# qhy991/llama.cpp-quant-gemm

Measured on AMD Instinct MI355X. Metric: effective TFLOPS + GB/s, Q4_0×Q8_1 GEMV M=1 N=K=4096; NMSE vs FP32, higher is better.
Workload: dtype int8; 1 GPU; q4_0_q8_1_gemv; M=1, N=4096, K=4096, rows_per_gpu=4096, weight_copies=64, parallelism=row-shard x1, launch=hipGraph, kernel_algo=1

## Files before the change

### include/qg/qg.h

```cpp
#ifndef QG_QG_H
#define QG_QG_H

#include <stddef.h>
#include <stdint.h>

#ifdef __cplusplus
extern "C" {
#endif

typedef struct ihipStream_t* qg_stream_t;

typedef enum {
    QG_TYPE_F32 = 0,
    QG_TYPE_F16 = 1,
    QG_TYPE_Q4_0 = 2,
    QG_TYPE_Q4_1 = 3,
    QG_TYPE_Q5_0 = 6,
    QG_TYPE_Q5_1 = 7,
    QG_TYPE_Q8_0 = 8,
    QG_TYPE_Q8_1 = 9,
    QG_TYPE_Q4_K = 12,
    QG_TYPE_Q6_K = 14,
    QG_TYPE_I32 = 26
} qg_type;
// ... 72 lines not shown
int qg_gemm_w8a16(const float* A, const void* B_q8_0, float* C, int M, int N, int K, qg_stream_t stream);
int qg_gemm_q4_0_fp32(const void* weight_q4_0, const float* activation, float* out, int M, int N, int K,
                      qg_stream_t stream);

int qg_gemm_w4a8_strided_batched(const void* A_q8_1, int64_t strideA, const void* B, int64_t strideB, float* C,
                                 int64_t strideC, int batch, int M, int N, int K, int wtype, qg_stream_t stream);

typedef struct {
    const void* A_q8_1;
    const void* B;
    float* C;
    int N;
    int ldc;
} qg_gemv_item;
int qg_gemm_w4a8_grouped(const qg_gemv_item* items, int count, int M, int K, int wtype, qg_stream_t stream);

int qg_gemm_w4a8_moe(const void* A_q8_1, int a_rows, const void* B_experts, int n_expert, const int32_t* ids,
                     int64_t ids_stride, float* C, int64_t ldc, int T, int n_used, int N, int K, int wtype,
                     qg_stream_t stream);
int qg_moe_config(int T, int n_used, int N, int K, int wtype, char* buf, size_t len);

size_t qg_gemm_w4a8_moe_prefill_workspace_size(int T, int n_used, int n_expert);
int qg_gemm_w4a8_moe_prefill(const void* A_q8_1, int a_rows, const void* B_experts, int n_expert, const int32_t* ids,
                             int64_t ids_stride, float* C, int64_t ldc, int T, int n_used, int N, int K, int wtype,
                             void* workspace, size_t workspace_bytes, qg_stream_t stream);
int qg_moe_prefill_config(int T, int n_used, int n_expert, int N, int K, int wtype, char* buf, size_t len);
int qg_debug_moe_prefill_plan(const int32_t* ids, int64_t ids_stride, int T, int n_used, int n_expert, int a_rows, int N,
                              int K, int wtype, int32_t* counts, int32_t* sorted, void* workspace,
                              size_t workspace_bytes, qg_stream_t stream);

// ... 95 lines not shown
```

### llama.cpp-quant-gemm_amd/csrc/qg_api.hip

```cpp
#include <string.h>

#include <initializer_list>

#include "../../include/qg/qg.h"
#include "qg_kernels.hpp"
#include "qg_moe_batch.hpp"
#include "qg_moe_prefill.hpp"
#include "qg_q4k.hpp"
#include "qg_q6k.hpp"

using namespace qg;

namespace qg {
int block_bytes(int t) {
    switch (t) {
        case QG_TYPE_Q4_0: return 18;
        case QG_TYPE_Q4_1: return 20;
        case QG_TYPE_Q5_0: return 22;
        case QG_TYPE_Q5_1: return 24;
        case QG_TYPE_Q8_0: return 34;
        case QG_TYPE_Q8_1: return 36;
        case QG_TYPE_Q4_K: return 144;
        case QG_TYPE_Q6_K: return 210;
    }
// ... 691 lines not shown

int qg_gemm_w4a8_tiled_act(const void* A_tiled, const void* B_tiled, float* C, int M, int N, int K, int wtype,
                           qg_stream_t stream) {
    return qg_gemm_w4a8_tiled_act_ldc(A_tiled, B_tiled, C, M, N, K, N, wtype, stream);
}

int qg_debug_sumi_tiled_act(const void* A_tiled, const void* B_tiled, int32_t* sumi, int M, int N, int K, int wtype,
                            qg_stream_t stream) {
    return tiled_sumi(LAY_TILED_ACT, A_tiled, B_tiled, sumi, M, N, K, wtype, stream);
}

int qg_debug_config_tiled_act(int M, int N, int K, int wtype, int sumi, char* buf, size_t len) {
    return describe_product(LAY_TILED_ACT, M, N, K, wtype, QG_ALGO_AUTO, sumi, buf, len);
}

int qg_gemm_w4a8_grouped(const qg_gemv_item* items, int count, int M, int K, int wtype, qg_stream_t stream) {
    if (count < 0 || M < 0 || (count > 0 && !items)) return QG_ERR_INVALID_ARG;
    if (K <= 0 || K % 32 != 0) return QG_ERR_BAD_K;
    if (!is_weight_type(wtype)) return QG_ERR_UNSUPPORTED;
    const hipStream_t st = (hipStream_t)stream;
    auto item_args = [&](const qg_gemv_item& it) {
        GemmArgs g = product_args(it.A_q8_1, it.B, it.C, M, it.N, K, wtype);
        if (it.ldc) g.ldc_m = it.ldc;
        return g;
    };
    bool one_launch = M > 0 && M <= 4;
    for (int i = 0; i < count; ++i) {
        const qg_gemv_item& it = items[i];
        if (it.N < 0 || it.ldc < 0 || (it.ldc != 0 && it.ldc < it.N)) return QG_ERR_INVALID_ARG;
        if (it.N == 0 || M == 0) continue;
        if (!it.A_q8_1 || !it.B || !it.C) return QG_ERR_INVALID_ARG;
        if (((uintptr_t)it.B & 1) != 0) return QG_ERR_ALIGN;
        const GemmArgs g = item_args(it);
        one_launch = one_launch && select_algo(g) == QG_ALGO_GEMV && gemv_eligible(g);
    }
    if (M == 0) return QG_OK;
    if (!one_launch) {
        for (int i = 0; i < count; ++i) {
            if (items[i].N == 0) continue;
            GemmArgs g = item_args(items[i]);
            const int rc = run_product(g, QG_ALGO_AUTO, st, false);
            if (rc != QG_OK) return rc;
        }
        return QG_OK;
    }
    for (int i0 = 0; i0 < count;) {
        GemvGroup grp = {};
        grp.M = M; grp.K = K;
        for (; i0 < count && grp.count < GEMV_GROUP_MAX; ++i0) {
            const qg_gemv_item& it = items[i0];
            if (it.N == 0) continue;
            grp.it[grp.count++] = GemvItemDesc{it.A_q8_1, it.B, it.C, it.N, it.ldc ? it.ldc : it.N};
        }
        if (grp.count == 0) break;
        const int rc = hip_status(launch_gemv(group_args(grp, wtype), st));
        if (rc != QG_OK) return rc;
    }
    return QG_OK;
}

int qg_gemm_w4a8(const void* A, const void* B, float* C, int M, int N, int K, int wtype, qg_stream_t stream) {
    return qg_gemm_w4a8_ex(A, B, C, M, N, K, wtype, QG_ALGO_AUTO, stream);
}

int qg_gemm_q4_0_q8_1_w4a8(const void* A_q8_1, const void* B_q4_0, float* C, int M, int N, int K,
                           qg_stream_t stream) {
    return qg_gemm_w4a8_ex(A_q8_1, B_q4_0, C, M, N, K, QG_TYPE_Q4_0, QG_ALGO_AUTO, stream);
}

int qg_gemm_q4_0_q8_1(const void* W, const void* A, float* out, int M, int N, int K, qg_stream_t s) {
    return weight_major(QG_TYPE_Q4_0, W, A, out, M, N, K, s);
}
int qg_gemm_q4_1_q8_1(const void* W, const void* A, float* out, int M, int N, int K, qg_stream_t s) {
    return weight_major(QG_TYPE_Q4_1, W, A, out, M, N, K, s);
// ... 155 lines not shown
```

### llama.cpp-quant-gemm_amd/csrc/qg_capture_fuse.hip

```cpp
#include <stdlib.h>

#include <algorithm>
#include <atomic>

#include "../../include/qg/qg.h"
#include "qg_capture_fuse.hpp"
#include "qg_kernels.hpp"

namespace qg {
namespace {
static_assert(fuse::MAX_ITEMS == GEMV_GROUP_MAX, "qg_capture_fuse.hpp and qg_kernels.hpp disagree on the group size");
std::atomic<int> g_fuse_mode{-1};
std::atomic<uint64_t> g_fuse_merged{0}, g_fuse_nodes{0};

int fuse_mode() {
    int m = g_fuse_mode.load(std::memory_order_relaxed);
    if (m >= 0) return m;
    const char* e = getenv("QG_CAPTURE_FUSE");
    m = e && e[0] == '0' && !e[1] ? 0 : e && e[0] == '2' && !e[1] ? 2 : 1;
    int unset = -1;
    g_fuse_mode.compare_exchange_strong(unset, m, std::memory_order_relaxed);
    return g_fuse_mode.load(std::memory_order_relaxed);
}

struct FuseRecord {
    bool valid = false;
    unsigned long long id = 0;
    hipGraphNode_t node = nullptr;
    int wtype = 0;
    GemvGroup grp = {};
    fuse::Group spans;
};
thread_local FuseRecord t_fuse;


bool fuse_candidate(const GemmArgs& g) {
    return g.batch == 1 && g.ldc_n == 1 && !g.sumi && !g.describe && !g.group && g.ain == AIN_Q8_1 && g.nbw == 0 &&
           g.lay == LAY_ROWS && g.M <= 4 && g.ldc_m >= 0 && g.ldc_m <= INT32_MAX;
}

bool fuse_class_enabled(const GemvNodeFill& nf, int M, int mode) {
    if (mode == 2) return true;
    return nf.one || M == 1;
}

hipError_t capture_gemv(const GemmArgs& g, hipStream_t st) {
// ... 11 lines not shown
        return cs == hipStreamCaptureStatusActive;
    };
    if (!capturing()) {
        r.valid = false;
        return launch_gemv(g, st);
    }
    const int mode = fuse_mode();
    const fuse::ItemSpans sp = fuse::item_spans(g.A, g.B, g.C, g.M, g.N, g.K, g.ldc_m, block_bytes(g.wtype));
    if (mode && r.valid && r.id == id && nd == 1 && deps[0] == r.node && r.grp.M == g.M && r.grp.K == g.K &&
        r.wtype == g.wtype && r.grp.count < GEMV_GROUP_MAX && fuse::can_join(r.spans, sp)) {
        GemvGroup grp = r.grp;
        grp.it[grp.count++] = GemvItemDesc{g.A, g.B, g.C, g.N, (int)g.ldc_m};
        GemvNodeFill nf;
        GemmArgs q = group_args(grp, g.wtype);
        q.node_fill = &nf;
        nf.p = hipKernelNodeParams{};
        hipError_t e = launch_gemv(q, st);
        if (e == hipSuccess && !(nf.p.func && fuse_class_enabled(nf, g.M, mode))) e = hipErrorNotSupported;
        if (e == hipSuccess) e = hipGraphKernelNodeSetParams(r.node, &nf.p);
        if (e == hipSuccess) {
            r.grp = grp;
            fuse::join(r.spans, sp);
            g_fuse_merged.fetch_add(1, std::memory_order_relaxed);
            return hipSuccess;
        }
        (void)hipGetLastError();
    }
    r.valid = false;
    const hipError_t e = launch_gemv(g, st);
    if (e != hipSuccess) return e;
    g_fuse_nodes.fetch_add(1, std::memory_order_relaxed);
    if (capturing() && nd == 1) {
        r.valid = true;
        r.id = id;
        r.node = deps[0];
        r.wtype = g.wtype;
        r.grp = GemvGroup{};
        r.grp.count = 1; r.grp.M = g.M; r.grp.K = g.K;
        r.grp.it[0] = GemvItemDesc{g.A, g.B, g.C, g.N, (int)g.ldc_m};
        r.spans.count = 0;
        fuse::join(r.spans, sp);
    }
    return hipSuccess;
}
}

hipError_t launch_or_merge_gemv(const GemmArgs& g, hipStream_t st) {
    return fuse_candidate(g) ? capture_gemv(g, st) : launch_gemv(g, st);
}

void set_capture_fusion(int on) { g_fuse_mode.store(on == 2 ? 2 : on ? 1 : 0, std::memory_order_relaxed); }
// ... 8 lines not shown
```

### llama.cpp-quant-gemm_amd/csrc/qg_gemv.hip

```cpp
#include "qg_gemv_impl.hpp"

namespace qg {

bool gemv_eligible(const GemmArgs& g) {
    switch (g.wtype) {
        case FMT_Q4_0: return ok_f<FMT_Q4_0>(g);
        case FMT_Q4_1: return ok_f<FMT_Q4_1>(g);
        case FMT_Q5_0: return ok_f<FMT_Q5_0>(g);
        case FMT_Q5_1: return ok_f<FMT_Q5_1>(g);
        case FMT_Q8_0: return ok_f<FMT_Q8_0>(g);
    }
    return false;
}

hipError_t launch_gemv(const GemmArgs& g, hipStream_t st) {
    switch (g.wtype) {
        case FMT_Q4_0: return gemv_launch_fmt<FMT_Q4_0>(g, st);
        case FMT_Q4_1: return gemv_launch_fmt<FMT_Q4_1>(g, st);
        case FMT_Q5_0: return gemv_launch_fmt<FMT_Q5_0>(g, st);
        case FMT_Q5_1: return gemv_launch_fmt<FMT_Q5_1>(g, st);
        case FMT_Q8_0: return gemv_launch_fmt<FMT_Q8_0>(g, st);
    }
    return hipErrorInvalidValue;
}
// ... 3 lines not shown
```

### llama.cpp-quant-gemm_amd/csrc/qg_gemv_kernel.hpp

```cpp
#pragma once
#include "qg_common.hpp"
#include "qg_kernels.hpp"
#include "qg_quant_block.hpp"

namespace qg {

constexpr uint32_t ACC_BIAS = 0x4B400000u;
constexpr float ACC_BIAS_F = 12582912.0f;

template <int F, int BPL> struct gemv_geom {
    static constexpr int BB = wfmt<F>::BB;
    static constexpr int UB = BPL * BB;
    static constexpr int UDW = UB / 4;
    static constexpr int REC_DW = 12 * BPL + 4;
};

template <int F> constexpr bool gemv_planes = F == FMT_Q4_0 || F == FMT_Q4_1;
template <int F> constexpr float gemv_cs = F == FMT_Q4_0 ? 8.0f : F == FMT_Q5_0 ? 16.0f : F == FMT_Q8_0 ? 0.0f : 1.0f;

template <int HI> __device__ __forceinline__ float mixmul(uint32_t h, float x) {
    float r;
    if constexpr (HI) asm("v_fma_mix_f32 %0, %1, %2, 0 op_sel:[1,0,0] op_sel_hi:[1,0,0]" : "=v"(r) : "v"(h), "v"(x));
    else asm("v_fma_mix_f32 %0, %1, %2, 0 op_sel_hi:[1,0,0]" : "=v"(r) : "v"(h), "v"(x));
    return r;
// ... 161 lines not shown
#pragma unroll
        for (int i = 0; i < 4; ++i) {
            const uint4 t = p[i];
            const uint32_t w[4] = {t.x, t.y, t.z, t.w};
#pragma unroll
            for (int j = 0; j < 4; ++j) {
                v[8 * i + 2 * j] = h2f(w[j] & 0xFFFFu);
                v[8 * i + 2 * j + 1] = h2f(w[j] >> 16);
            }
        }
    }
}

typedef uint32_t u32x4_a4 __attribute__((ext_vector_type(4), aligned(4)));
typedef uint32_t u32x2_a4 __attribute__((ext_vector_type(2), aligned(4)));

#ifndef QG_GEMV_PRE_MT
#define QG_GEMV_PRE_MT 0
#endif
template <int F> constexpr int gemv_pre_mt = QG_GEMV_PRE_MT ? QG_GEMV_PRE_MT : (F == FMT_Q4_0 || F == FMT_Q4_1) ? 2 : 4;
#ifndef QG_GEMV_ACT2
#define QG_GEMV_ACT2 1
#endif
template <int F, int MT, int BPL, int LPR, int WGS, bool SUMI, int AIN, bool NT, bool PRE, int ONEU, int TPW = 1>
__device__ __forceinline__ void gemv_body(const uint32_t* __restrict__ A, const uint8_t* __restrict__ B, long sA, long sB,
                                          int M, int N, int K, float* __restrict__ C, long sC, long ldc_m, long ldc_n,
                                          int32_t* __restrict__ sumi_out, int tile_in = -1) {
    static_assert(TPW == 1 || ONEU == 1, "several tiles per workgroup: the one-unit form only");
    constexpr int NUN = ONEU > 1 ? ONEU : 1;
    using G = gemv_geom<F, BPL>;
    A = reinterpret_cast<const uint32_t*>(reinterpret_cast<const uint8_t*>(A) + blockIdx.y * sA);
    B += blockIdx.y * sB;
    C += blockIdx.y * sC;
    constexpr int RPW = 64 / LPR;
    constexpr int RPB = (WGS / 64) * RPW;
    extern __shared__ __attribute__((aligned(16))) uint32_t lds[];

    const int nb = K / QK;
    const int U = nb / BPL;
    const int tid = threadIdx.x;
    const int lane = tid & 63;
    const int lir = lane % LPR;
    const int tile = tile_in >= 0 ? tile_in : gridDim.x <= 512 ? xcd_tile(blockIdx.x, gridDim.x) : (int)blockIdx.x;
    int rows[TPW];
    bool rows_ok[TPW];
    const uint8_t* wrows[TPW];
#pragma unroll
    for (int t = 0; t < TPW; ++t) {
        rows[t] = (tile * TPW + t) * RPB + (tid >> 6) * RPW + lane / LPR;
        rows_ok[t] = rows[t] < N;
        wrows[t] = B + (long)(rows_ok[t] ? rows[t] : 0) * ((long)U * G::UB);
    }
    const int row = rows[0];
    const bool row_ok = rows_ok[0];
    auto load_unit = [&](uint32_t (&dst)[G::UDW], int u, int t = 0) {
        const uint32_t* p = reinterpret_cast<const uint32_t*>(wrows[t] + (long)((rows_ok[t] && u < U) ? u : 0) * G::UB);
        if constexpr (NT) {
#pragma unroll
// ... 183 lines not shown
#define QG_GEMV_TPW 1
#endif
#ifndef QG_GEMVG_TPW
#define QG_GEMVG_TPW 2
#endif
#ifndef QG_GEMV_MTGW
#define QG_GEMV_MTGW 256
#endif
#ifndef QG_GEMV_MTTPW
#define QG_GEMV_MTTPW 2
#endif
#ifndef QG_GEMVG_WDIV
#define QG_GEMVG_WDIV 2
#endif
template <int F, int MT, int BPL, int LPR, int WGS, bool PRE, int ONEU, int TPW = 1>
__global__ __launch_bounds__(WGS) void gemvg_kernel(const GemvGroup grp) {
    constexpr int RPB = (WGS / 64) * (64 / LPR) * TPW;
    const int item = blockIdx.y;
    const int tile = gridDim.x <= 512 ? xcd_tile(blockIdx.x, gridDim.x) : (int)blockIdx.x;
    const GemvItemDesc d = grp.it[item];
    if (!grp.full && tile * RPB >= d.N) return;
    gemv_body<F, MT, BPL, LPR, WGS, false, AIN_Q8_1, false, PRE, ONEU, TPW>(
        reinterpret_cast<const uint32_t*>(d.A), reinterpret_cast<const uint8_t*>(d.B), 0, 0, grp.M, d.N, grp.K,
        d.C, 0, d.ldc, 1, nullptr, tile);
}

#ifndef QG_GEMV_NU
#define QG_GEMV_NU 1
#endif
#ifndef QG_GEMV_NU_MT
#define QG_GEMV_NU_MT 1
#endif


template <int F, int BPL> inline size_t gemv_lds_bytes(int M, int K) {
    return (size_t)M * (K / QK / BPL) * gemv_geom<F, BPL>::REC_DW * 4;
}

template <int F, int BPL>
inline bool gemv_shape_ok(const GemmArgs& g) {
    if (g.M < 1 || g.M > 8) return false;
    if (g.K % (QK * BPL) != 0) return false;
    const int aal = g.ain == AIN_Q8_1 ? 3 : 15;
    if (((uintptr_t)g.B & 3) != 0 || ((uintptr_t)g.A & aal) != 0) return false;
    if (g.batch > 1 && ((g.sB & 3) != 0 || (g.sA & aal) != 0)) return false;
    if (g.sumi && g.ain != AIN_Q8_1) return false;
    if (g.M > 2 && gemv_lds_bytes<F, BPL>(g.M, g.K) > 96 * 1024) return false;
    return true;
}

template <int F, int MT, int BPL, int LPR, int WGS, bool SUMI, int AIN = AIN_Q8_1, bool NT = false, bool PRE = (MT <= 2)>
hipError_t gemv_launch(const GemmArgs& g, hipStream_t st) {
    constexpr int RPB = (WGS / 64) * (64 / LPR);
    const size_t lds = gemv_lds_bytes<F, BPL>(g.M, g.K);
    const int grid = (g.N + RPB - 1) / RPB;
    const bool one = g.K / QK / BPL <= LPR;
    constexpr bool NU_OK = QG_GEMV_NU && MT <= QG_GEMV_NU_MT && F == FMT_Q4_0;
    const int nu_all = (g.K / QK / BPL + LPR - 1) / LPR;
    const int nu = one ? 1 : !NU_OK ? 0 : nu_all <= 2 ? 2 : nu_all <= 4 ? 4 : 0;
    const bool m1 = MT == 1 && PRE && !NT && g.M == 1 && g.batch == 1 && g.ldc_n == 1;
    const bool shrt = !m1 && !NT && g.batch == 1 && g.ldc_m <= INT32_MAX && g.ldc_n <= INT32_MAX;
    const int oneu = m1 ? nu : shrt ? ((nu > 1 && !(NU_OK && MT > 1)) ? 0 : nu) : (int)one;
    if (g.group && (SUMI || AIN != AIN_Q8_1 || NT || MT > 4)) return hipErrorInvalidValue;
    if (g.describe) {
        describe_kernel(g, "gemv F=%d MT=%d BPL=%d LPR=%d WGS=%d AIN=%d NT=%d PRE=%d ONEU=%d SIG=%s grid=%dx%d", F, MT, BPL,
                        LPR, WGS, AIN, (int)NT, (int)(one ? PRE : (PRE && MT <= (shrt && !oneu ? gemv_pre_mt<F> : 2))), oneu,
                        m1 ? "m1" : shrt ? "short" : "full",
                        grid, g.batch);
        return hipSuccess;
    }
    if constexpr (!SUMI && AIN == AIN_Q8_1 && !NT && MT <= 4) {
        if (g.group) {
            const GemvGroup& grp0 = *static_cast<const GemvGroup*>(g.group);
            auto go = [&](auto GWc, auto TPc) -> hipError_t {
                constexpr int GW = decltype(GWc)::value, TP = decltype(TPc)::value;
                GemvGroup grp = grp0;
                constexpr int RPBG = (GW / 64) * (64 / LPR);
                const int rpw = one ? RPBG * TP : RPBG;
                int tiles = 0, tmin = INT32_MAX;
                for (int i = 0; i < grp.count; ++i) {
                    const int t = (grp.it[i].N + rpw - 1) / rpw;
                    tiles = std::max(tiles, t);
                    tmin = std::min(tmin, t);
                }
                auto kg = one ? gemvg_kernel<F, MT, BPL, LPR, GW, PRE, true, TP>
                              : gemvg_kernel<F, MT, BPL, LPR, GW, PRE && (MT <= 2), false>;
                if (lds > 64 * 1024) {
                    hipError_t e = hipFuncSetAttribute((const void*)kg, hipFuncAttributeMaxDynamicSharedMemorySize, (int)lds);
                    if (e != hipSuccess) return e;
                }
                if (g.node_fill) g.node_fill->p = hipKernelNodeParams{};
                if (tiles == 0 || grp.count == 0) return hipSuccess;
                grp.full = tiles == tmin ? 1 : 0;
                if (GemvNodeFill* nf = g.node_fill) {
                    nf->grp = grp;
                    nf->argv[0] = &nf->grp;
                    nf->one = one ? 1 : 0;
                    nf->p.func = (void*)kg;
                    nf->p.gridDim = dim3(tiles, grp.count);
                    nf->p.blockDim = dim3(GW);
                    nf->p.sharedMemBytes = (unsigned)lds;
                    nf->p.kernelParams = nf->argv;
                    return hipSuccess;
                }
                hipLaunchKernelGGL(kg, dim3(tiles, grp.count), dim3(GW), lds, st, grp);
                return hipGetLastError();
            };
            constexpr bool MTW = QG_GEMV_MTGW > 0 && MT >= 2;
            constexpr int GWH = MTW ? (QG_GEMV_MTGW < WGS ? QG_GEMV_MTGW : WGS) : WGS / QG_GEMVG_WDIV;
            constexpr int TPH = MTW ? QG_GEMV_MTTPW : QG_GEMVG_TPW;
            if constexpr (GWH < WGS && GWH >= 64) {
                const int rpw_full = one ? RPB * QG_GEMVG_TPW : RPB;
                int nmax = 0;
                for (int i = 0; i < grp0.count; ++i) nmax = std::max(nmax, grp0.it[i].N);
                if ((nmax + rpw_full - 1) / rpw_full <= device_cus())
                    return go(std::integral_constant<int, GWH>{}, std::integral_constant<int, TPH>{});
            }
            return go(std::integral_constant<int, WGS>{}, std::integral_constant<int, QG_GEMVG_TPW>{});
        }
    }
    if (m1) {
// ... 23 lines not shown
        }
        void* out = SUMI ? (void*)g.sumi : (void*)g.C;
        hipLaunchKernelGGL(ks, dim3(grid), dim3(WGS), lds, st, (const uint32_t*)g.A, (const uint8_t*)g.B, g.M, g.N, g.K, out,
                           (int)g.ldc_m, (int)g.ldc_n);
        return hipGetLastError();
    }
#ifndef QG_GEMVB_WDIV
#define QG_GEMVB_WDIV 2
#endif
    constexpr bool MTB = QG_GEMV_MTGW > 0 && MT >= 2;
    constexpr int GWB = MTB ? (QG_GEMV_MTGW < WGS ? QG_GEMV_MTGW : WGS) : WGS / QG_GEMVB_WDIV;
    constexpr int TPB = MTB ? QG_GEMV_MTTPW : QG_GEMV_TPW;
    if constexpr (GWB < WGS && GWB >= 64 && !SUMI && !NT) {
        constexpr int GW = GWB, RPBB = (GW / 64) * (64 / LPR) * TPB;
        if (one && g.batch > 1 && grid <= device_cus()) {
            auto kb = gemv_kernel<F, MT, BPL, LPR, GW, SUMI, AIN, NT, PRE, true, TPB>;
            if (lds > 64 * 1024) {
                hipError_t e = hipFuncSetAttribute((const void*)kb, hipFuncAttributeMaxDynamicSharedMemorySize, (int)lds);
                if (e != hipSuccess) return e;
            }
            hipLaunchKernelGGL(kb, dim3((g.N + RPBB - 1) / RPBB, g.batch), dim3(GW), lds, st, (const uint32_t*)g.A,
                               (const uint8_t*)g.B, g.sA, g.sB, g.M, g.N, g.K, g.C, g.sC, g.ldc_m, g.ldc_n, g.sumi);
            return hipGetLastError();
        }
    }
    constexpr bool tpw_ok = !SUMI && !NT && QG_GEMV_TPW > 1;
    const bool multi = tpw_ok && one && g.batch > 1;
    auto kfn = multi ? gemv_kernel<F, MT, BPL, LPR, WGS, SUMI, AIN, NT, PRE, true, tpw_ok ? QG_GEMV_TPW : 1>
             : one   ? gemv_kernel<F, MT, BPL, LPR, WGS, SUMI, AIN, NT, PRE, true>
                     : gemv_kernel<F, MT, BPL, LPR, WGS, SUMI, AIN, NT, PRE && (MT <= 2), false>;
    if (lds > 64 * 1024) {
        hipError_t e = hipFuncSetAttribute((const void*)kfn, hipFuncAttributeMaxDynamicSharedMemorySize, (int)lds);
        if (e != hipSuccess) return e;
    }
    const int gx = multi ? (g.N + RPB * QG_GEMV_TPW - 1) / (RPB * QG_GEMV_TPW) : grid;
    hipLaunchKernelGGL(kfn, dim3(gx, g.batch), dim3(WGS), lds, st, (const uint32_t*)g.A, (const uint8_t*)g.B, g.sA,
                       g.sB, g.M, g.N, g.K, g.C, g.sC, g.ldc_m, g.ldc_n, g.sumi);
    return hipGetLastError();
}

}
```

### llama.cpp-quant-gemm_amd/csrc/qg_kernels.hpp

```cpp
#pragma once
#include <hip/hip_runtime.h>
#include <stddef.h>
#include <stdint.h>
#include <stdio.h>

#include <atomic>
#include <mutex>

namespace qg {

enum : int { AIN_Q8_1 = 0, AIN_F32 = 1, AIN_F16_FUSED = 2 };

enum : int { LAY_ROWS = 0, LAY_TILED = 1, LAY_TILED_ACT = 2 };
constexpr int ACT_TILE = 16;
constexpr int ACT_STG = ACT_TILE * 4 * 36;

struct GemmArgs {
    const void* A = nullptr;
    int ain = AIN_Q8_1;
    const void* B = nullptr;
    int lay = 0;
    int nbw = 0;
    float* C = nullptr;
    int32_t* sumi = nullptr;
    int M = 0, N = 0, K = 0;
    int wtype = 0;
    long ldc_m = 0, ldc_n = 1;
    int batch = 1;
    long sA = 0, sB = 0, sC = 0;
    void* ws = nullptr;
    size_t ws_bytes = 0;
    const void* group = nullptr;
    char* describe = nullptr;
    size_t describe_len = 0;
    struct GemvNodeFill* node_fill = nullptr;
};

constexpr int GEMV_GROUP_MAX = 64;
struct GemvItemDesc {
    const void* A;
    const void* B;
    float* C;
    int N, ldc;
};
struct GemvGroup {
    int count, M, K, full;
    GemvItemDesc it[GEMV_GROUP_MAX];
};
inline GemmArgs group_args(const GemvGroup& grp, int wtype) {
    GemmArgs g;
    g.A = grp.it[0].A; g.B = grp.it[0].B; g.C = grp.it[0].C; g.M = grp.M; g.K = grp.K; g.wtype = wtype;
    for (int i = 0; i < grp.count; ++i) g.N = grp.it[i].N > g.N ? grp.it[i].N : g.N;
    g.ldc_m = grp.it[0].ldc; g.ldc_n = 1;
    g.group = &grp;
    return g;
}
struct GemvNodeFill {
    hipKernelNodeParams p;
    GemvGroup grp;
    void* argv[1];
    int one;
};

inline hipError_t set_max_lds_once(const void* fn, int bytes, std::atomic<unsigned long long>& done) {
    int dev = 0;
    if (hipGetDevice(&dev) != hipSuccess) return hipErrorInvalidDevice;
    const unsigned long long bit = dev < 64 ? 1ull << dev : 0ull;
    if (bit && (done.load(std::memory_order_acquire) & bit)) return hipSuccess;
    const hipError_t e = hipFuncSetAttribute(fn, hipFuncAttributeMaxDynamicSharedMemorySize, bytes);
    if (e == hipSuccess && bit) done.fetch_or(bit, std::memory_order_acq_rel);
    return e;
}

int device_cus();

void describe_kernel(const GemmArgs& g, const char* fmt, ...);
template <class... V> void describe_line(char* buf, size_t len, const char* fmt, V... v) {
// ... 67 lines not shown
```

### llama.cpp-quant-gemm_amd/quant_gemm/__init__.py

```python
from __future__ import annotations

import ctypes

import torch

from . import _lib

__version__ = "0.1.0"

QK4_0 = 32
QK8_1 = 32
BLOCK_Q4_0_BYTES = 18
BLOCK_Q8_1_BYTES = 36

Q4_0, Q4_1, Q5_0, Q5_1, Q8_0, Q8_1 = 2, 3, 6, 7, 8, 9
Q4_K = 12
Q6_K = 14
BLOCK_BYTES = {Q4_0: 18, Q4_1: 20, Q5_0: 22, Q5_1: 24, Q8_0: 34, Q8_1: 36, Q4_K: 144, Q6_K: 210}
ALGO_AUTO, ALGO_GEMV, ALGO_MFMA, ALGO_GENERIC, ALGO_RAGGED = 0, 1, 2, 3, 4
WEIGHT_TYPES = (Q4_0, Q4_1, Q5_0, Q5_1, Q8_0)
GEMM_WEIGHT_TYPES = WEIGHT_TYPES + (Q4_K, Q6_K)


def block_elems(qtype: int) -> int:
# ... 561 lines not shown
    return _config("qg_debug_config_tiled_act", M, N, K, wtype, int(sumi))


def debug_config_tiled(M: int, N: int, K: int, wtype: int = Q4_0, sumi: bool = False) -> str:
    return _config("qg_debug_config_tiled", M, N, K, wtype, int(sumi))


def select_algo(M: int, N: int, K: int, wtype: int = Q4_0) -> int:
    return _lib.load().qg_select_algo(M, N, K, wtype)


def set_capture_fusion(on) -> None:
    _lib.load().qg_set_capture_fusion(int(on))


def capture_fusion_stats() -> "tuple[int, int]":
    merged, nodes = ctypes.c_uint64(0), ctypes.c_uint64(0)
    _lib.load().qg_capture_fusion_stats(ctypes.byref(merged), ctypes.byref(nodes))
    return int(merged.value), int(nodes.value)


def version() -> str:
    return _lib.load().qg_version().decode()


_lib.load()

__all__ = [
    "quantize_q4_0", "quantize_q8_1", "gemm_q4_0_q8_1", "dequantize_q4_0",
    "QK4_0", "QK8_1", "BLOCK_Q4_0_BYTES", "BLOCK_Q8_1_BYTES",
    "quantize", "dequantize", "gemm_w4a8", "gemm_q4_1_q8_1", "gemm_q5_0_q8_1", "gemm_q5_1_q8_1",
    "gemm_w4a8_batched", "debug_sumi", "debug_config", "select_algo", "version",
    "gemm_w4a8_f32", "gemm_q4_0_fp16_fused", "quantize_q8_1_f16_fused", "gemm_w8a8", "gemm_q8_0_q8_1",
    "gemm_w4a16", "gemm_w8a16", "gemm_q4_0_fp32",
    "tile_weights", "gemm_w4a8_tiled", "debug_sumi_tiled", "debug_config_tiled",
    "quantize_q8_1_tiled", "tile_activations", "gemm_w4a8_tiled_act", "debug_sumi_tiled_act", "debug_config_tiled_act",
    "Q4_0", "Q4_1", "Q5_0", "Q5_1", "Q8_0", "Q8_1", "Q4_K", "Q6_K", "block_elems",
    "set_capture_fusion", "capture_fusion_stats",
    "gemm_w4a8_moe", "moe_config",
    "gemm_w4a8_moe_prefill", "moe_prefill_workspace_size", "moe_prefill_config", "debug_moe_prefill_plan",
    "gemm_w4a8_moe_batch", "moe_batch_workspace_size", "moe_batch_config",
]
```

### llama.cpp-quant-gemm_amd/quant_gemm/_lib.py

```python
from __future__ import annotations

import ctypes
import os

import torch

HERE = os.path.dirname(os.path.abspath(__file__))
LIB_PATH = os.path.join(HERE, "libqg_hip.so")
CSRC = os.path.join(os.path.dirname(HERE), "csrc")

QG_OK = 0
STATUS = {0: "ok", -1: "invalid argument", -2: "K must be a positive multiple of 32",
          -3: "unsupported type or algorithm for this shape", -4: "pointer misaligned for the block format",
          -5: "HIP launch error"}

P, I, I64, SZ = ctypes.c_void_p, ctypes.c_int, ctypes.c_int64, ctypes.c_size_t
SIGNATURES = {
    "qg_gemm_w4a8": ([P, P, P, I, I, I, I, P], I),
    "qg_gemm_w4a8_ex": ([P, P, P, I, I, I, I, I, P], I),
    "qg_gemm_q4_0_q8_1_w4a8": ([P, P, P, I, I, I, P], I),
    "qg_gemm_w4a8_ldc": ([P, P, P, I, I, I, I64, I, I, P], I),
    "qg_debug_config": ([I, I, I, I, I, I, ctypes.c_char_p, SZ], I),
    "qg_gemm_w4a8_strided_batched": ([P, I64, P, I64, P, I64, I, I, I, I, I, P], I),
    "qg_gemm_w4a8_grouped": ([P, I, I, I, I, P], I),
    "qg_gemm_w4a8_moe": ([P, I, P, I, P, I64, P, I64, I, I, I, I, I, P], I),
    "qg_moe_config": ([I, I, I, I, I, ctypes.c_char_p, SZ], I),
    "qg_gemm_w4a8_moe_prefill_workspace_size": ([I, I, I], SZ),
    "qg_gemm_w4a8_moe_prefill": ([P, I, P, I, P, I64, P, I64, I, I, I, I, I, P, SZ, P], I),
    "qg_moe_prefill_config": ([I, I, I, I, I, I, ctypes.c_char_p, SZ], I),
    "qg_debug_moe_prefill_plan": ([P, I64, I, I, I, I, I, I, I, P, P, P, SZ, P], I),
    "qg_gemm_w4a8_moe_batch_workspace_size": ([I, I, I], SZ),
    "qg_gemm_w4a8_moe_batch": ([P, I, P, I, P, I64, P, I64, I, I, I, I, I, P, SZ, P], I),
    "qg_moe_batch_config": ([I, I, I, I, I, I, ctypes.c_char_p, SZ], I),
    "qg_gemm_w4a8_workspace_size": ([I, I, I, I], SZ),
    "qg_gemm_w4a8_ws": ([P, P, P, I, I, I, I, P, SZ, P], I),
    "qg_repack_weights_bytes": ([I, I, I], SZ),
    "qg_repack_weights": ([P, P, I, I, I, P], I),
    "qg_gemm_w4a8_prepacked_workspace_size": ([I, I], SZ),
    "qg_gemm_w4a8_prepacked": ([P, P, P, I, I, I, I, P, SZ, P], I),
# ... 102 lines not shown
```

Measured before the change: 22.08 TFLOPS.

## Lower affine-strided GEMV groups to batched launch and slim grouped kernel args

When every item in a grouped GEMV shares N and ldc and its A, B, C pointers sit at constant strides, the group is launched as a strided-batched GEMV instead of the per-item descriptor kernel. This is gated by a mode setting and by size conditions, and it also applies inside graph capture fusion, with a fallback when setting the node parameters fails. The grouped kernel now takes scalar args plus an item array that is read with one vector load, and XCD tile remapping is driven by a flag. The change adds a describe/config API and an environment switch, at the cost of extra host-side stride checks and more code paths.

```diff
diff --git a/include/qg/qg.h b/include/qg/qg.h
--- a/include/qg/qg.h
+++ b/include/qg/qg.h
@@ -110,6 +110,10 @@
     int ldc;
 } qg_gemv_item;
 int qg_gemm_w4a8_grouped(const qg_gemv_item* items, int count, int M, int K, int wtype, qg_stream_t stream);
+
+void qg_set_group_affine(int mode);
+
+int qg_group_config(const qg_gemv_item* items, int count, int M, int K, int wtype, char* buf, size_t len);
 
 int qg_gemm_w4a8_moe(const void* A_q8_1, int a_rows, const void* B_experts, int n_expert, const int32_t* ids,
                      int64_t ids_stride, float* C, int64_t ldc, int T, int n_used, int N, int K, int wtype,
diff --git a/llama.cpp-quant-gemm_amd/csrc/qg_api.hip b/llama.cpp-quant-gemm_amd/csrc/qg_api.hip
--- a/llama.cpp-quant-gemm_amd/csrc/qg_api.hip
+++ b/llama.cpp-quant-gemm_amd/csrc/qg_api.hip
@@ -729,11 +729,11 @@
     return describe_product(LAY_TILED_ACT, M, N, K, wtype, QG_ALGO_AUTO, sumi, buf, len);
 }
 
-int qg_gemm_w4a8_grouped(const qg_gemv_item* items, int count, int M, int K, int wtype, qg_stream_t stream) {
+static int run_grouped(const qg_gemv_item* items, int count, int M, int K, int wtype, hipStream_t st, char* describe,
+                       size_t describe_len) {
     if (count < 0 || M < 0 || (count > 0 && !items)) return QG_ERR_INVALID_ARG;
     if (K <= 0 || K % 32 != 0) return QG_ERR_BAD_K;
     if (!is_weight_type(wtype)) return QG_ERR_UNSUPPORTED;
-    const hipStream_t st = (hipStream_t)stream;
     auto item_args = [&](const qg_gemv_item& it) {
         GemmArgs g = product_args(it.A_q8_1, it.B, it.C, M, it.N, K, wtype);
         if (it.ldc) g.ldc_m = it.ldc;
@@ -749,8 +749,15 @@
         const GemmArgs g = item_args(it);
         one_launch = one_launch && select_algo(g) == QG_ALGO_GEMV && gemv_eligible(g);
     }
-    if (M == 0) return QG_OK;
+    if (M == 0) {
+        describe_line(describe, describe_len, "%s", "none");
+        return QG_OK;
+    }
     if (!one_launch) {
+        if (describe) {
+            describe_line(describe, describe_len, "%s", "items: one qg_gemm_w4a8 launch per item");
+            return QG_OK;
+        }
         for (int i = 0; i < count; ++i) {
             if (items[i].N == 0) continue;
             GemmArgs g = item_args(items[i]);
@@ -759,6 +766,7 @@
         }
         return QG_OK;
     }
+    describe_line(describe, describe_len, "%s", "none");
     for (int i0 = 0; i0 < count;) {
         GemvGroup grp = {};
         grp.M = M; grp.K = K;
@@ -768,11 +776,26 @@
             grp.it[grp.count++] = GemvItemDesc{it.A_q8_1, it.B, it.C, it.N, it.ldc ? it.ldc : it.N};
         }
         if (grp.count == 0) break;
-        const int rc = hip_status(launch_gemv(group_args(grp, wtype), st));
-        if (rc != QG_OK) return rc;
+        GemmArgs q = group_args(grp, wtype);
+        q.describe = describe;
+        q.describe_len = describe_len;
+        const int rc = hip_status(launch_gemv(q, st));
+        if (rc != QG_OK || describe) return rc;
     }
     return QG_OK;
 }
+
+int qg_gemm_w4a8_grouped(const qg_gemv_item* items, int count, int M, int K, int wtype, qg_stream_t stream) {
+    return run_grouped(items, count, M, K, wtype, (hipStream_t)stream, nullptr, 0);
+}
+
+int qg_group_config(const qg_gemv_item* items, int count, int M, int K, int wtype, char* buf, size_t len) {
+    if (!buf || len == 0) return QG_ERR_INVALID_ARG;
+    buf[0] = 0;
+    return run_grouped(items, count, M, K, wtype, nullptr, buf, len);
+}
+
+void qg_set_group_affine(int mode) { set_group_affine(mode); }
 
 int qg_gemm_w4a8(const void* A, const void* B, float* C, int M, int N, int K, int wtype, qg_stream_t stream) {
     return qg_gemm_w4a8_ex(A, B, C, M, N, K, wtype, QG_ALGO_AUTO, stream);
diff --git a/llama.cpp-quant-gemm_amd/csrc/qg_capture_fuse.hip b/llama.cpp-quant-gemm_amd/csrc/qg_capture_fuse.hip
--- a/llama.cpp-quant-gemm_amd/csrc/qg_capture_fuse.hip
+++ b/llama.cpp-quant-gemm_amd/csrc/qg_capture_fuse.hip
@@ -30,6 +30,7 @@
     int wtype = 0;
     GemvGroup grp = {};
     fuse::Group spans;
+    bool no_affine = false;
 };
 thread_local FuseRecord t_fuse;
 
@@ -71,10 +72,21 @@
         GemvNodeFill nf;
         GemmArgs q = group_args(grp, g.wtype);
         q.node_fill = &nf;
+        if (r.no_affine) q.affine = -1;
         nf.p = hipKernelNodeParams{};
         hipError_t e = launch_gemv(q, st);
         if (e == hipSuccess && !(nf.p.func && fuse_class_enabled(nf, g.M, mode))) e = hipErrorNotSupported;
-        if (e == hipSuccess) e = hipGraphKernelNodeSetParams(r.node, &nf.p);
+        if (e == hipSuccess) {
+            e = hipGraphKernelNodeSetParams(r.node, &nf.p);
+            if (e != hipSuccess && nf.affine) {
+                (void)hipGetLastError();
+                r.no_affine = true;
+                q.affine = -1;
+                e = launch_gemv(q, st);
+                if (e == hipSuccess && !nf.p.func) e = hipErrorNotSupported;
+                if (e == hipSuccess) e = hipGraphKernelNodeSetParams(r.node, &nf.p);
+            }
+        }
         if (e == hipSuccess) {
             r.grp = grp;
             fuse::join(r.spans, sp);
@@ -92,6 +104,7 @@
         r.id = id;
         r.node = deps[0];
         r.wtype = g.wtype;
+        r.no_affine = false;
         r.grp = GemvGroup{};
         r.grp.count = 1; r.grp.M = g.M; r.grp.K = g.K;
         r.grp.it[0] = GemvItemDesc{g.A, g.B, g.C, g.N, (int)g.ldc_m};
diff --git a/llama.cpp-quant-gemm_amd/csrc/qg_gemv.hip b/llama.cpp-quant-gemm_amd/csrc/qg_gemv.hip
--- a/llama.cpp-quant-gemm_amd/csrc/qg_gemv.hip
+++ b/llama.cpp-quant-gemm_amd/csrc/qg_gemv.hip
@@ -1,6 +1,22 @@
+#include <stdlib.h>
+
 #include "qg_gemv_impl.hpp"
 
 namespace qg {
+
+static std::atomic<int> g_affine_mode{-1};
+
+int group_affine_mode() {
+    int m = g_affine_mode.load(std::memory_order_relaxed);
+    if (m >= 0) return m;
+    const char* e = getenv("QG_GROUP_AFFINE");
+    m = e && e[0] == '0' && !e[1] ? 0 : e && e[0] == '2' && !e[1] ? 2 : 1;
+    int unset = -1;
+    g_affine_mode.compare_exchange_strong(unset, m, std::memory_order_relaxed);
+    return g_affine_mode.load(std::memory_order_relaxed);
+}
+
+void set_group_affine(int mode) { g_affine_mode.store(mode == 2 ? 2 : mode ? 1 : 0, std::memory_order_relaxed); }
 
 bool gemv_eligible(const GemmArgs& g) {
     switch (g.wtype) {
diff --git a/llama.cpp-quant-gemm_amd/csrc/qg_gemv_kernel.hpp b/llama.cpp-quant-gemm_amd/csrc/qg_gemv_kernel.hpp
--- a/llama.cpp-quant-gemm_amd/csrc/qg_gemv_kernel.hpp
+++ b/llama.cpp-quant-gemm_amd/csrc/qg_gemv_kernel.hpp
@@ -1,5 +1,8 @@
 #pragma once
+#include <assert.h>
+
 #include "qg_common.hpp"
+#include "qg_group_affine.hpp"
 #include "qg_kernels.hpp"
 #include "qg_quant_block.hpp"
 
@@ -7,6 +10,8 @@
 
 constexpr uint32_t ACC_BIAS = 0x4B400000u;
 constexpr float ACC_BIAS_F = 12582912.0f;
+
+__host__ __device__ constexpr int gemv_tiles(int N, int rpw) { return (int)(((unsigned)N + (unsigned)rpw - 1u) / (unsigned)rpw); }
 
 template <int F, int BPL> struct gemv_geom {
     static constexpr int BB = wfmt<F>::BB;
@@ -199,6 +204,11 @@
 
 typedef uint32_t u32x4_a4 __attribute__((ext_vector_type(4), aligned(4)));
 typedef uint32_t u32x2_a4 __attribute__((ext_vector_type(2), aligned(4)));
+typedef uint32_t u32x8_a16 __attribute__((ext_vector_type(8), aligned(16)));
+template <class T> __device__ __forceinline__ T* global_ptr(uint32_t lo, uint32_t hi) {
+    typedef T __attribute__((address_space(1))) * G;
+    return (T*)(G)((uint64_t)lo | (uint64_t)hi << 32);
+}
 
 #ifndef QG_GEMV_PRE_MT
 #define QG_GEMV_PRE_MT 0
@@ -226,7 +236,8 @@
     const int tid = threadIdx.x;
     const int lane = tid & 63;
     const int lir = lane % LPR;
-    const int tile = tile_in >= 0 ? tile_in : gridDim.x <= 512 ? xcd_tile(blockIdx.x, gridDim.x) : (int)blockIdx.x;
+    const int ntile = gemv_tiles(N, RPB * TPW);
+    const int tile = tile_in >= 0 ? tile_in : ntile <= 512 ? xcd_tile(blockIdx.x, ntile) : (int)blockIdx.x;
     int rows[TPW];
     bool rows_ok[TPW];
     const uint8_t* wrows[TPW];
@@ -440,15 +451,21 @@
 #define QG_GEMVG_WDIV 2
 #endif
 template <int F, int MT, int BPL, int LPR, int WGS, bool PRE, int ONEU, int TPW = 1>
-__global__ __launch_bounds__(WGS) void gemvg_kernel(const GemvGroup grp) {
+__global__ __launch_bounds__(WGS) void gemvg_kernel(int M, int K, int flags, int tiles, const GemvItems items) {
     constexpr int RPB = (WGS / 64) * (64 / LPR) * TPW;
-    const int item = blockIdx.y;
-    const int tile = gridDim.x <= 512 ? xcd_tile(blockIdx.x, gridDim.x) : (int)blockIdx.x;
-    const GemvItemDesc d = grp.it[item];
-    if (!grp.full && tile * RPB >= d.N) return;
+    static_assert(sizeof(GemvItemDesc) == 32 && offsetof(GemvItemDesc, N) == 24 && offsetof(GemvItemDesc, ldc) == 28, "");
+    const u32x8_a16 r = *reinterpret_cast<const u32x8_a16*>(&items.it[blockIdx.y]);
+    GemvItemDesc d;
+    d.A = global_ptr<const void>(r[0], r[1]);
+    d.B = global_ptr<const void>(r[2], r[3]);
+    d.C = global_ptr<float>(r[4], r[5]);
+    d.N = (int)r[6];
+    d.ldc = (int)r[7];
+    const int tile = (flags & GEMVG_XCD) ? xcd_tile(blockIdx.x, tiles) : (int)blockIdx.x;
+    if (!(flags & GEMVG_FULL) && tile * RPB >= d.N) return;
     gemv_body<F, MT, BPL, LPR, WGS, false, AIN_Q8_1, false, PRE, ONEU, TPW>(
-        reinterpret_cast<const uint32_t*>(d.A), reinterpret_cast<const uint8_t*>(d.B), 0, 0, grp.M, d.N, grp.K,
-        d.C, 0, d.ldc, 1, nullptr, tile);
+        reinterpret_cast<const uint32_t*>(d.A), reinterpret_cast<const uint8_t*>(d.B), 0, 0, M, d.N, K,
+        d.C, 0, d.ldc, 1, nullptr, tile & INT32_MAX);
 }
 
 #ifndef QG_GEMV_NU
@@ -475,11 +492,15 @@
     return true;
 }
 
+inline bool group_affine_class_enabled(bool one, int MT, bool small_n, int count, int mode) {
+    if (mode == 2) return true;
+    return one && MT == 1 && small_n && count >= 8;
+}
+
 template <int F, int MT, int BPL, int LPR, int WGS, bool SUMI, int AIN = AIN_Q8_1, bool NT = false, bool PRE = (MT <= 2)>
 hipError_t gemv_launch(const GemmArgs& g, hipStream_t st) {
     constexpr int RPB = (WGS / 64) * (64 / LPR);
     const size_t lds = gemv_lds_bytes<F, BPL>(g.M, g.K);
-    const int grid = (g.N + RPB - 1) / RPB;
     const bool one = g.K / QK / BPL <= LPR;
     constexpr bool NU_OK = QG_GEMV_NU && MT <= QG_GEMV_NU_MT && F == FMT_Q4_0;
     const int nu_all = (g.K / QK / BPL + LPR - 1) / LPR;
@@ -488,7 +509,25 @@
     const bool shrt = !m1 && !NT && g.batch == 1 && g.ldc_m <= INT32_MAX && g.ldc_n <= INT32_MAX;
     const int oneu = m1 ? nu : shrt ? ((nu > 1 && !(NU_OK && MT > 1)) ? 0 : nu) : (int)one;
     if (g.group && (SUMI || AIN != AIN_Q8_1 || NT || MT > 4)) return hipErrorInvalidValue;
-    if (g.describe) {
+    auto grid_x = [&](int rpw) {
+        const int gx = (g.N + rpw - 1) / rpw;
+        assert(gx == gemv_tiles(g.N, rpw));
+        return gx;
+    };
+    const int grid = grid_x(RPB);
+    auto fill_batch = [&](const void* fn, dim3 grd, int block) {
+        GemvNodeFill* nf = g.node_fill;
+        nf->p = hipKernelNodeParams{};
+        nf->set_batch(g);
+        nf->one = one ? 1 : 0;
+        nf->p.func = const_cast<void*>(fn);
+        nf->p.gridDim = grd;
+        nf->p.blockDim = dim3(block);
+        nf->p.sharedMemBytes = (unsigned)lds;
+        nf->p.kernelParams = nf->argv;
+        return hipSuccess;
+    };
+    if (g.describe && !g.group && !g.affine) {
         describe_kernel(g, "gemv F=%d MT=%d BPL=%d LPR=%d WGS=%d AIN=%d NT=%d PRE=%d ONEU=%d SIG=%s grid=%dx%d", F, MT, BPL,
                         LPR, WGS, AIN, (int)NT, (int)(one ? PRE : (PRE && MT <= (shrt && !oneu ? gemv_pre_mt<F> : 2))), oneu,
                         m1 ? "m1" : shrt ? "short" : "full",
@@ -498,16 +537,35 @@
     if constexpr (!SUMI && AIN == AIN_Q8_1 && !NT && MT <= 4) {
         if (g.group) {
             const GemvGroup& grp0 = *static_cast<const GemvGroup*>(g.group);
+            affine::Strides as;
+            const int amode = group_affine_mode();
+            if (amode && g.affine >= 0 && grp0.count >= 2 && group_affine_class_enabled(one, MT, g.N <= 16 * device_cus(), grp0.count, amode) &&
+                affine::group_affine(grp0.it, grp0.count, 3, 15, &as)) {
+                GemmArgs b = g;
+                b.group = nullptr;
+                b.affine = 1;
+                b.A = grp0.it[0].A; b.B = grp0.it[0].B; b.C = grp0.it[0].C;
+                b.N = grp0.it[0].N; b.ldc_m = grp0.it[0].ldc; b.ldc_n = 1;
+                b.batch = grp0.count;
+                b.sA = (long)as.a; b.sB = (long)as.b; b.sC = (long)(as.c / 4);
+                return gemv_launch<F, MT, BPL, LPR, WGS, SUMI, AIN, NT, PRE>(b, st);
+            }
             auto go = [&](auto GWc, auto TPc) -> hipError_t {
                 constexpr int GW = decltype(GWc)::value, TP = decltype(TPc)::value;
-                GemvGroup grp = grp0;
                 constexpr int RPBG = (GW / 64) * (64 / LPR);
                 const int rpw = one ? RPBG * TP : RPBG;
                 int tiles = 0, tmin = INT32_MAX;
-                for (int i = 0; i < grp.count; ++i) {
-                    const int t = (grp.it[i].N + rpw - 1) / rpw;
+                for (int i = 0; i < grp0.count; ++i) {
+                    const int t = (grp0.it[i].N + rpw - 1) / rpw;
                     tiles = std::max(tiles, t);
                     tmin = std::min(tmin, t);
+                }
+                const int full = tiles == tmin ? 1 : 0;
+                if (g.describe) {
+                    describe_kernel(g, "gemvg F=%d MT=%d BPL=%d LPR=%d WGS=%d PRE=%d ONEU=%d TPW=%d full=%d grid=%dx%d", F, MT,
+                                    BPL, LPR, GW, (int)(one ? PRE : PRE && MT <= 2), (int)one, one ? TP : 1, full, tiles,
+                                    grp0.count);
+                    return hipSuccess;
                 }
                 auto kg = one ? gemvg_kernel<F, MT, BPL, LPR, GW, PRE, true, TP>
                               : gemvg_kernel<F, MT, BPL, LPR, GW, PRE && (MT <= 2), false>;
@@ -516,21 +574,25 @@
                     if (e != hipSuccess) return e;
                 }
                 if (g.node_fill) g.node_fill->p = hipKernelNodeParams{};
-                if (tiles == 0 || grp.count == 0) return hipSuccess;
-                grp.full = tiles == tmin ? 1 : 0;
-                if (GemvNodeFill* nf = g.node_fill) {
-                    nf->grp = grp;
-                    nf->argv[0] = &nf->grp;
-                    nf->one = one ? 1 : 0;
-                    nf->p.func = (void*)kg;
-                    nf->p.gridDim = dim3(tiles, grp.count);
-                    nf->p.blockDim = dim3(GW);
-                    nf->p.sharedMemBytes = (unsigned)lds;
-                    nf->p.kernelParams = nf->argv;
-                    return hipSuccess;
-                }
-                hipLaunchKernelGGL(kg, dim3(tiles, grp.count), dim3(GW), lds, st, grp);
-                return hipGetLastError();
+                if (tiles == 0 || grp0.count == 0) return hipSuccess;
+                GemvNodeFill local;
+                GemvNodeFill* nf = g.node_fill ? g.node_fill : &local;
+                nf->p = hipKernelNodeParams{};
+                nf->grp = grp0;
+                nf->grp.full = full;
+                nf->flags = (full ? GEMVG_FULL : 0) | (tiles <= 512 ? GEMVG_XCD : 0);
+                nf->tiles = tiles;
+                nf->argv[0] = &nf->grp.M; nf->argv[1] = &nf->grp.K; nf->argv[2] = &nf->flags; nf->argv[3] = &nf->tiles;
+                nf->argv[4] = nf->grp.it;
+                nf->one = one ? 1 : 0;
+                nf->affine = 0;
+                nf->p.func = (void*)kg;
+                nf->p.gridDim = dim3(tiles, grp0.count);
+                nf->p.blockDim = dim3(GW);
+                nf->p.sharedMemBytes = (unsigned)lds;
+                nf->p.kernelParams = nf->argv;
+                if (g.node_fill) return hipSuccess;
+                return hipLaunchKernel(nf->p.func, nf->p.gridDim, nf->p.blockDim, nf->argv, lds, st);
             };
             constexpr bool MTW = QG_GEMV_MTGW > 0 && MT >= 2;
             constexpr int GWH = MTW ? (QG_GEMV_MTGW < WGS ? QG_GEMV_MTGW : WGS) : WGS / QG_GEMVG_WDIV;
@@ -584,18 +646,30 @@
     if constexpr (GWB < WGS && GWB >= 64 && !SUMI && !NT) {
         constexpr int GW = GWB, RPBB = (GW / 64) * (64 / LPR) * TPB;
         if (one && g.batch > 1 && grid <= device_cus()) {
+            if (g.describe) {
+                describe_kernel(g, "gemvb F=%d MT=%d BPL=%d LPR=%d WGS=%d PRE=%d ONEU=1 TPW=%d grid=%dx%d", F, MT, BPL, LPR, GW,
+                                (int)PRE, TPB, grid_x(RPBB), g.batch);
+                return hipSuccess;
+            }
             auto kb = gemv_kernel<F, MT, BPL, LPR, GW, SUMI, AIN, NT, PRE, true, TPB>;
             if (lds > 64 * 1024) {
                 hipError_t e = hipFuncSetAttribute((const void*)kb, hipFuncAttributeMaxDynamicSharedMemorySize, (int)lds);
                 if (e != hipSuccess) return e;
             }
-            hipLaunchKernelGGL(kb, dim3((g.N + RPBB - 1) / RPBB, g.batch), dim3(GW), lds, st, (const uint32_t*)g.A,
+            if (g.affine && g.node_fill) return fill_batch((const void*)kb, dim3(grid_x(RPBB), g.batch), GW);
+            hipLaunchKernelGGL(kb, dim3(grid_x(RPBB), g.batch), dim3(GW), lds, st, (const uint32_t*)g.A,
                                (const uint8_t*)g.B, g.sA, g.sB, g.M, g.N, g.K, g.C, g.sC, g.ldc_m, g.ldc_n, g.sumi);
             return hipGetLastError();
         }
     }
     constexpr bool tpw_ok = !SUMI && !NT && QG_GEMV_TPW > 1;
     const bool multi = tpw_ok && one && g.batch > 1;
+    const int gx = multi ? grid_x(RPB * QG_GEMV_TPW) : grid;
+    if (g.describe) {
+        describe_kernel(g, "gemvb F=%d MT=%d BPL=%d LPR=%d WGS=%d PRE=%d ONEU=%d TPW=%d grid=%dx%d", F, MT, BPL, LPR, WGS,
+                        (int)(one ? PRE : PRE && MT <= 2), (int)one, multi ? QG_GEMV_TPW : 1, gx, g.batch);
+        return hipSuccess;
+    }
     auto kfn = multi ? gemv_kernel<F, MT, BPL, LPR, WGS, SUMI, AIN, NT, PRE, true, tpw_ok ? QG_GEMV_TPW : 1>
              : one   ? gemv_kernel<F, MT, BPL, LPR, WGS, SUMI, AIN, NT, PRE, true>
                      : gemv_kernel<F, MT, BPL, LPR, WGS, SUMI, AIN, NT, PRE && (MT <= 2), false>;
@@ -603,7 +677,7 @@
         hipError_t e = hipFuncSetAttribute((const void*)kfn, hipFuncAttributeMaxDynamicSharedMemorySize, (int)lds);
         if (e != hipSuccess) return e;
     }
-    const int gx = multi ? (g.N + RPB * QG_GEMV_TPW - 1) / (RPB * QG_GEMV_TPW) : grid;
+    if (g.affine && g.node_fill) return fill_batch((const void*)kfn, dim3(gx, g.batch), WGS);
     hipLaunchKernelGGL(kfn, dim3(gx, g.batch), dim3(WGS), lds, st, (const uint32_t*)g.A, (const uint8_t*)g.B, g.sA,
                        g.sB, g.M, g.N, g.K, g.C, g.sC, g.ldc_m, g.ldc_n, g.sumi);
     return hipGetLastError();
diff --git a/llama.cpp-quant-gemm_amd/csrc/qg_group_affine.hpp b/llama.cpp-quant-gemm_amd/csrc/qg_group_affine.hpp
--- /dev/null
+++ b/llama.cpp-quant-gemm_amd/csrc/qg_group_affine.hpp
@@ -0,0 +1,49 @@
+#pragma once
+#include <stddef.h>
+#include <stdint.h>
+
+namespace qg {
+namespace affine {
+
+struct Strides {
+    intptr_t a, b, c;
+};
+
+inline bool ptr_diff(const void* q, const void* p, intptr_t* d) {
+    const uintptr_t uq = (uintptr_t)q, up = (uintptr_t)p;
+    if (uq >= up) {
+        if (uq - up > (uintptr_t)INTPTR_MAX) return false;
+        *d = (intptr_t)(uq - up);
+    } else {
+        if (up - uq > (uintptr_t)INTPTR_MAX) return false;
+        *d = -(intptr_t)(up - uq);
+    }
+    return true;
+}
+
+template <class Item>
+inline bool group_affine(const Item* it, int count, uintptr_t a_mask, uintptr_t b_mask, Strides* s) {
+    if (!it || count < 1) return false;
+    Strides st = {0, 0, 0};
+    if (count > 1 && !(ptr_diff(it[1].A, it[0].A, &st.a) && ptr_diff(it[1].B, it[0].B, &st.b) &&
+                       ptr_diff(it[1].C, it[0].C, &st.c)))
+        return false;
+    if (((uintptr_t)st.a & a_mask) != 0 || ((uintptr_t)st.b & b_mask) != 0 || ((uintptr_t)st.c & 3) != 0) return false;
+    for (int i = 1; i < count; ++i) {
+        if (it[i].N != it[0].N || it[i].ldc != it[0].ldc) return false;
+        intptr_t da, db, dc;
+        if (!(ptr_diff(it[i].A, it[i - 1].A, &da) && ptr_diff(it[i].B, it[i - 1].B, &db) &&
+              ptr_diff(it[i].C, it[i - 1].C, &dc)))
+            return false;
+        if (da != st.a || db != st.b || dc != st.c) return false;
+    }
+    intptr_t t;
+    if (!(ptr_diff(it[count - 1].A, it[0].A, &t) && ptr_diff(it[count - 1].B, it[0].B, &t) &&
+          ptr_diff(it[count - 1].C, it[0].C, &t)))
+        return false;
+    *s = st;
+    return true;
+}
+
+}
+}
diff --git a/llama.cpp-quant-gemm_amd/csrc/qg_kernels.hpp b/llama.cpp-quant-gemm_amd/csrc/qg_kernels.hpp
--- a/llama.cpp-quant-gemm_amd/csrc/qg_kernels.hpp
+++ b/llama.cpp-quant-gemm_amd/csrc/qg_kernels.hpp
@@ -34,6 +34,7 @@
     char* describe = nullptr;
     size_t describe_len = 0;
     struct GemvNodeFill* node_fill = nullptr;
+    int affine = 0;
 };
 
 constexpr int GEMV_GROUP_MAX = 64;
@@ -43,10 +44,15 @@
     float* C;
     int N, ldc;
 };
+struct GemvItems {
+    GemvItemDesc it[GEMV_GROUP_MAX];
+};
 struct GemvGroup {
     int count, M, K, full;
     GemvItemDesc it[GEMV_GROUP_MAX];
 };
+static_assert(sizeof(GemvItems) == sizeof(GemvGroup::it), "the kernel argument is read from GemvGroup::it");
+enum : int { GEMVG_FULL = 1, GEMVG_XCD = 2 };
 inline GemmArgs group_args(const GemvGroup& grp, int wtype) {
     GemmArgs g;
     g.A = grp.it[0].A; g.B = grp.it[0].B; g.C = grp.it[0].C; g.M = grp.M; g.K = grp.K; g.wtype = wtype;
@@ -58,9 +64,23 @@
 struct GemvNodeFill {
     hipKernelNodeParams p;
     GemvGroup grp;
-    void* argv[1];
+    int flags, tiles;
+    struct Batch {
+        const uint32_t* A; const uint8_t* B; long sA, sB; int M, N, K; float* C; long sC, ldc_m, ldc_n; int32_t* sumi;
+    } sb;
+    void* argv[12];
     int one;
+    int affine;
+    void set_batch(const GemmArgs& g) {
+        sb = Batch{(const uint32_t*)g.A, (const uint8_t*)g.B, g.sA, g.sB, g.M, g.N, g.K, g.C, g.sC, g.ldc_m, g.ldc_n, nullptr};
+        void* a[12] = {&sb.A, &sb.B, &sb.sA, &sb.sB, &sb.M, &sb.N, &sb.K, &sb.C, &sb.sC, &sb.ldc_m, &sb.ldc_n, &sb.sumi};
+        for (int i = 0; i < 12; ++i) argv[i] = a[i];
+        affine = 1;
+    }
 };
+
+int group_affine_mode();
+void set_group_affine(int mode);
 
 inline hipError_t set_max_lds_once(const void* fn, int bytes, std::atomic<unsigned long long>& done) {
     int dev = 0;
diff --git a/llama.cpp-quant-gemm_amd/quant_gemm/__init__.py b/llama.cpp-quant-gemm_amd/quant_gemm/__init__.py
--- a/llama.cpp-quant-gemm_amd/quant_gemm/__init__.py
+++ b/llama.cpp-quant-gemm_amd/quant_gemm/__init__.py
@@ -599,6 +599,18 @@
     _lib.load().qg_set_capture_fusion(int(on))
 
 
+def set_group_affine(mode) -> None:
+    _lib.load().qg_set_group_affine(int(mode))
+
+
+def group_config(items, M: int, K: int, wtype: int = Q4_0) -> str:
+    n = len(items)
+    arr = (_GemvItem * max(n, 1))(*[_GemvItem(*it) for it in items])
+    buf = ctypes.create_string_buffer(256)
+    _lib.check(_lib.load().qg_group_config(arr, n, M, K, wtype, buf, len(buf)), "group_config")
+    return buf.value.decode()
+
+
 def capture_fusion_stats() -> "tuple[int, int]":
     merged, nodes = ctypes.c_uint64(0), ctypes.c_uint64(0)
     _lib.load().qg_capture_fusion_stats(ctypes.byref(merged), ctypes.byref(nodes))
@@ -621,7 +633,7 @@
     "tile_weights", "gemm_w4a8_tiled", "debug_sumi_tiled", "debug_config_tiled",
     "quantize_q8_1_tiled", "tile_activations", "gemm_w4a8_tiled_act", "debug_sumi_tiled_act", "debug_config_tiled_act",
     "Q4_0", "Q4_1", "Q5_0", "Q5_1", "Q8_0", "Q8_1", "Q4_K", "Q6_K", "block_elems",
-    "set_capture_fusion", "capture_fusion_stats",
+    "set_capture_fusion", "capture_fusion_stats", "set_group_affine", "group_config",
     "gemm_w4a8_moe", "moe_config",
     "gemm_w4a8_moe_prefill", "moe_prefill_workspace_size", "moe_prefill_config", "debug_moe_prefill_plan",
     "gemm_w4a8_moe_batch", "moe_batch_workspace_size", "moe_batch_config",
diff --git a/llama.cpp-quant-gemm_amd/quant_gemm/_lib.py b/llama.cpp-quant-gemm_amd/quant_gemm/_lib.py
--- a/llama.cpp-quant-gemm_amd/quant_gemm/_lib.py
+++ b/llama.cpp-quant-gemm_amd/quant_gemm/_lib.py
@@ -23,6 +23,8 @@
     "qg_debug_config": ([I, I, I, I, I, I, ctypes.c_char_p, SZ], I),
     "qg_gemm_w4a8_strided_batched": ([P, I64, P, I64, P, I64, I, I, I, I, I, P], I),
     "qg_gemm_w4a8_grouped": ([P, I, I, I, I, P], I),
+    "qg_group_config": ([P, I, I, I, I, ctypes.c_char_p, SZ], I),
+    "qg_set_group_affine": ([I], None),
     "qg_gemm_w4a8_moe": ([P, I, P, I, P, I64, P, I64, I, I, I, I, I, P], I),
     "qg_moe_config": ([I, I, I, I, I, ctypes.c_char_p, SZ], I),
     "qg_gemm_w4a8_moe_prefill_workspace_size": ([I, I, I], SZ),
```

After: 22.85 TFLOPS, median of 6. 3.5% higher.
